# tailhook/ciruela

Measured on AMD Instinct MI355X. Metric: GiB/s block-hashed (device-resident, blocks in HBM) at 1/2/4/8 MI355X, higher is better.
Workload: dtype u64; 1 GPU; config2: 1048576 x 32768 B blocks per GPU (32 GiB), splitmix64, device-resident; blocks_per_gpu=1048576, block_size=32768, entry_point=cir_hash_chunks_dev, loader=lds-dma, parallelism=range-split x1, no collective

## Files before the change

ciruela_amd/csrc/blake2b_dev.hpp:

```cpp
#pragma once
#include <hip/hip_runtime.h>
#include <stdint.h>

#include <type_traits>

namespace cir {
namespace dev {

__device__ __forceinline__ uint32_t lo32(uint64_t x) { return (uint32_t)x; }
__device__ __forceinline__ uint32_t hi32(uint64_t x) { return (uint32_t)(x >> 32); }
__device__ __forceinline__ uint64_t mk64(uint32_t lo, uint32_t hi) {
  return ((uint64_t)hi << 32) | lo;
}
typedef uint32_t u32x2_t __attribute__((ext_vector_type(2)));
__device__ __forceinline__ uint64_t mk64_pair(uint32_t lo, uint32_t hi) {
  const u32x2_t v = {lo, hi};
  return __builtin_bit_cast(uint64_t, v);
}

__device__ __forceinline__ uint64_t xor3(uint64_t a, uint64_t b, uint64_t c) {
  return mk64(__builtin_amdgcn_bitop3_b32(lo32(a), lo32(b), lo32(c), 0x96),
              __builtin_amdgcn_bitop3_b32(hi32(a), hi32(b), hi32(c), 0x96));
}

#define CIR_IV0 0x6a09e667f3bcc908ULL
#define CIR_IV1 0xbb67ae8584caa73bULL
#define CIR_IV2 0x3c6ef372fe94f82bULL
#define CIR_IV3 0xa54ff53a5f1d36f1ULL
#define CIR_IV4 0x510e527fade682d1ULL
#define CIR_IV5 0x9b05688c2b3e6c1fULL
#define CIR_IV6 0x1f83d9abfb41bd6bULL
#define CIR_IV7 0x5be0cd19137e2179ULL
#define CIR_P0_256 0x01010020ULL

__device__ __forceinline__ void sched_fence() { __builtin_amdgcn_sched_barrier(0); }

template <int N>
__device__ __forceinline__ uint64_t rotr_lh(uint32_t l, uint32_t h) {
  if constexpr (N == 32)
    return mk64(h, l);
  else if constexpr (N < 32)
    return mk64(__builtin_amdgcn_alignbit(h, l, N), __builtin_amdgcn_alignbit(l, h, N));
  else
    return mk64(__builtin_amdgcn_alignbit(l, h, N - 32), __builtin_amdgcn_alignbit(h, l, N - 32));
}

#define CIR_XOR4(P, Q)                                            \
  tl0 = lo32(P##0) ^ lo32(Q##0); th0 = hi32(P##0) ^ hi32(Q##0);  \
  tl1 = lo32(P##1) ^ lo32(Q##1); th1 = hi32(P##1) ^ hi32(Q##1);  \
  tl2 = lo32(P##2) ^ lo32(Q##2); th2 = hi32(P##2) ^ hi32(Q##2);  \
  tl3 = lo32(P##3) ^ lo32(Q##3); th3 = hi32(P##3) ^ hi32(Q##3);
#define CIR_ROT4(P, N)              \
  P##0 = rotr_lh<N>(tl0, th0);      \
  P##1 = rotr_lh<N>(tl1, th1);      \
  P##2 = rotr_lh<N>(tl2, th2);      \
  P##3 = rotr_lh<N>(tl3, th3);
#define CIR_ADD4(P, Q) P##0 = P##0 + (Q##0); P##1 = P##1 + (Q##1); P##2 = P##2 + (Q##2); P##3 = P##3 + (Q##3);

__device__ __forceinline__ void g4(uint64_t& a0, uint64_t& a1, uint64_t& a2, uint64_t& a3,
                                   uint64_t& b0, uint64_t& b1, uint64_t& b2, uint64_t& b3,
                                   uint64_t& c0, uint64_t& c1, uint64_t& c2, uint64_t& c3,
                                   uint64_t& d0, uint64_t& d1, uint64_t& d2, uint64_t& d3,
                                   uint64_t x0, uint64_t x1, uint64_t x2, uint64_t x3,
                                   uint64_t y0, uint64_t y1, uint64_t y2, uint64_t y3) {
  uint32_t tl0, tl1, tl2, tl3, th0, th1, th2, th3;
  CIR_ADD4(a, x) CIR_ADD4(a, b)
  sched_fence();
  CIR_XOR4(d, a) CIR_ROT4(d, 32)
  sched_fence();
  CIR_ADD4(c, d)
  sched_fence();
  CIR_XOR4(b, c)
  sched_fence();
  CIR_ROT4(b, 24) CIR_ADD4(a, y) CIR_ADD4(a, b)
  sched_fence();
  CIR_XOR4(d, a)
  sched_fence();
  CIR_ROT4(d, 16) CIR_ADD4(c, d)
  sched_fence();
  CIR_XOR4(b, c)
  sched_fence();
  CIR_ROT4(b, 63)
}

#define CIR_ROUND_SM(s0, s1, s2, s3, s4, s5, s6, s7, s8, s9, s10, s11, s12, s13, s14, s15)    \
  g4(v0, v1, v2, v3, v4, v5, v6, v7, v8, v9, v10, v11, v12, v13, v14, v15, m[s0], m[s2], m[s4], \
     m[s6], m[s1], m[s3], m[s5], m[s7]);                                                       \
  g4(v0, v1, v2, v3, v5, v6, v7, v4, v10, v11, v8, v9, v15, v12, v13, v14, m[s8], m[s10],       \
     m[s12], m[s14], m[s9], m[s11], m[s13], m[s15]);

struct NoHook {
  __device__ __forceinline__ void operator()() const {}
};

template <typename Hook = NoHook>
__device__ __forceinline__ void compress_sm(uint64_t h[8], const uint64_t m[16], uint64_t t,
                                            bool last, Hook after_col0 = Hook()) {
  uint64_t v0 = h[0], v1 = h[1], v2 = h[2], v3 = h[3];
  uint64_t v4 = h[4], v5 = h[5], v6 = h[6], v7 = h[7];
  uint64_t v8 = CIR_IV0, v9 = CIR_IV1, v10 = CIR_IV2, v11 = CIR_IV3;
  uint64_t v12 = CIR_IV4 ^ t, v13 = CIR_IV5;
  uint64_t v14 = last ? ~CIR_IV6 : CIR_IV6, v15 = CIR_IV7;
  g4(v0, v1, v2, v3, v4, v5, v6, v7, v8, v9, v10, v11, v12, v13, v14, v15, m[0], m[2], m[4],
     m[6], m[1], m[3], m[5], m[7]);
  if constexpr (!std::is_same_v<Hook, NoHook>) {
    asm volatile("" : "+v"(v0), "+v"(v1), "+v"(v2), "+v"(v3), "+v"(v4), "+v"(v5), "+v"(v6),
                 "+v"(v7));
    asm volatile("" : "+v"(v8), "+v"(v9), "+v"(v10), "+v"(v11), "+v"(v12), "+v"(v13),
                 "+v"(v14), "+v"(v15));
    sched_fence();
    after_col0();
    sched_fence();
  }
  g4(v0, v1, v2, v3, v5, v6, v7, v4, v10, v11, v8, v9, v15, v12, v13, v14, m[8], m[10],
     m[12], m[14], m[9], m[11], m[13], m[15]);
  CIR_ROUND_SM(14, 10, 4, 8, 9, 15, 13, 6, 1, 12, 0, 2, 11, 7, 5, 3)
  CIR_ROUND_SM(11, 8, 12, 0, 5, 2, 15, 13, 10, 14, 3, 6, 7, 1, 9, 4)
  CIR_ROUND_SM(7, 9, 3, 1, 13, 12, 11, 14, 2, 6, 5, 10, 4, 0, 15, 8)
  CIR_ROUND_SM(9, 0, 5, 7, 2, 4, 10, 15, 14, 1, 11, 12, 6, 8, 3, 13)
  CIR_ROUND_SM(2, 12, 6, 10, 0, 11, 8, 3, 4, 13, 7, 5, 15, 14, 1, 9)
  CIR_ROUND_SM(12, 5, 1, 15, 14, 13, 4, 10, 0, 7, 6, 3, 9, 2, 8, 11)
  CIR_ROUND_SM(13, 11, 7, 14, 12, 1, 3, 9, 5, 0, 15, 4, 8, 6, 2, 10)
  CIR_ROUND_SM(6, 15, 14, 9, 11, 3, 0, 8, 12, 2, 13, 7, 1, 4, 10, 5)
  CIR_ROUND_SM(10, 2, 8, 4, 7, 6, 1, 5, 15, 11, 9, 14, 3, 12, 13, 0)
  CIR_ROUND_SM(0, 1, 2, 3, 4, 5, 6, 7, 8, 9, 10, 11, 12, 13, 14, 15)
  CIR_ROUND_SM(14, 10, 4, 8, 9, 15, 13, 6, 1, 12, 0, 2, 11, 7, 5, 3)
  sched_fence();
  h[0] = xor3(h[0], v0, v8);
  h[1] = xor3(h[1], v1, v9);
  h[2] = xor3(h[2], v2, v10);
  h[3] = xor3(h[3], v3, v11);
  h[4] = xor3(h[4], v4, v12);
  h[5] = xor3(h[5], v5, v13);
  h[6] = xor3(h[6], v6, v14);
  h[7] = xor3(h[7], v7, v15);
}

__device__ __forceinline__ void compress(uint64_t h[8], const uint64_t m[16], uint64_t t,
                                         bool last) {
  compress_sm(h, m, t, last);
}

__device__ __forceinline__ void init_state(uint64_t h[8]) {
  h[0] = CIR_IV0 ^ CIR_P0_256;
  h[1] = CIR_IV1;
  h[2] = CIR_IV2;
  h[3] = CIR_IV3;
  h[4] = CIR_IV4;
  h[5] = CIR_IV5;
  h[6] = CIR_IV6;
  h[7] = CIR_IV7;
}

__device__ __forceinline__ void load_line16(uint64_t m[16], const uint8_t* p) {
  const uint4* q = reinterpret_cast<const uint4*>(p);
#pragma unroll
  for (int k = 0; k < 8; ++k) {
    const uint4 x = q[k];
    m[2 * k] = mk64(x.x, x.y);
    m[2 * k + 1] = mk64(x.z, x.w);
  }
}

__device__ __forceinline__ void load_line_safe(uint64_t m[16], const uint8_t* p, uint32_t n) {
  const bool al4 = (reinterpret_cast<uintptr_t>(p) & 3u) == 0;
#pragma unroll
  for (int w = 0; w < 32; ++w) {
    uint32_t x = 0;
    const uint32_t b0 = 4u * w;
    if (al4 && b0 + 4u <= n) {
      x = *reinterpret_cast<const uint32_t*>(p + b0);
    } else {
#pragma unroll
      for (int k = 0; k < 4; ++k)
        if (b0 + k < n) x |= (uint32_t)p[b0 + k] << (8 * k);
    }
    if (w & 1)
      m[w >> 1] |= (uint64_t)x << 32;
    else
      m[w >> 1] = x;
  }
}

__device__ __forceinline__ void load_line_any(uint64_t m[16], const uint8_t* p, uint64_t i,
                                              uint64_t nfull, uint32_t rem, bool al16) {
  const uint8_t* q = p + (i << 7);
  if (al16 && i < nfull) {
    load_line16(m, q);
  } else {
    uint32_t n = i < nfull ? 128u : rem;
    asm volatile("" : "+v"(n));
    load_line_safe(m, q, n);
  }
}

__device__ __forceinline__ void hash_chain(const uint8_t* p, uint64_t len, uint64_t h[8]) {
  init_state(h);
  const uint32_t nfull = (uint32_t)(len >> 7);
  const uint32_t rem = (uint32_t)(len & 127u);
  const uint32_t total = nfull + ((rem != 0u || len == 0) ? 1u : 0u);
  const bool al16 = (reinterpret_cast<uintptr_t>(p) & 15u) == 0;
  uint64_t m[16];
  for (uint32_t i = 0; i < total; ++i) {
    load_line_any(m, p, i, nfull, rem, al16);
    const bool last = i + 1 == total;
    compress(h, m, last ? len : (uint64_t)(i + 1) << 7, last);
  }
}

// ... 256 lines not shown
```

ciruela_amd/csrc/kernels.hip:

```cpp
#include "kernels.hpp"

#include <algorithm>
#include <atomic>
#include <cstdlib>

#include "blake2b_dev.hpp"
#include "uniform.hpp"
#include "sha512_dev.hpp"

namespace cir {
namespace dev {

static inline unsigned grid_for(uint64_t n, uint64_t per) { return (unsigned)((n + per - 1) / per); }

__global__ __launch_bounds__(kThreads, 5) void k_uniform_glds(const uint8_t* __restrict__ data,
                                                               uint64_t bs, uint32_t lines,
                                                               uint8_t* __restrict__ out) {
  __shared__ __attribute__((aligned(16))) uint8_t lds[kWaves * kWaveLds];
  const uint32_t wave = __builtin_amdgcn_readfirstlane(threadIdx.x >> 6);
  const uint64_t blk0 = ((uint64_t)blockIdx.x * kWaves + wave) * 64u;
  uniform_glds_wave(data + blk0 * bs, bs, lines, out + blk0 * 32u, lds + wave * kWaveLds);
}

__global__ __launch_bounds__(kThreads, 4) void k_chunks(const uint8_t* __restrict__ data,
                                                         uint64_t nbytes, uint64_t bs,
                                                         uint32_t lines, uint64_t nfull,
                                                         uint32_t ngen_wg,
                                                         uint8_t* __restrict__ out) {
  __shared__ __attribute__((aligned(16))) uint8_t lds[kWaves * kWaveLds];
  if (blockIdx.x < ngen_wg) {
    if (threadIdx.x != 0) return;
    uint64_t h[8];
    hash_chain_al16(data + nfull * bs, nbytes - nfull * bs, h);
    store_digest(out + nfull * 32u, h);
    return;
  }
  const uint32_t wave = __builtin_amdgcn_readfirstlane(threadIdx.x >> 6);
  const uint64_t blk0 = ((uint64_t)(blockIdx.x - ngen_wg) * kWaves + wave) * 64u;
  if (blk0 >= nfull) return;
  const uint64_t nv = nfull - blk0;
  if (nv >= 64)
    uniform_glds_wave(data + blk0 * bs, bs, lines, out + blk0 * 32u, lds + wave * kWaveLds);
  else
    uniform_glds_wave<true>(data + blk0 * bs, bs, lines, out + blk0 * 32u, lds + wave * kWaveLds,
                            (uint32_t)nv);
}

__global__ __launch_bounds__(kThreads, 4) void k_uniform_direct(const uint8_t* __restrict__ data,
                                                                 uint64_t bs, uint32_t lines,
                                                                 uint8_t* __restrict__ out) {
  const uint64_t b = (uint64_t)blockIdx.x * kThreads + threadIdx.x;
  const uint8_t* p = data + b * bs;
  uint64_t h[8];
  init_state(h);
  uint64_t ma[16], mb[16];
  load_line16(ma, p);
  for (uint32_t i = 0; i < lines; i += 2) {
    if (i + 1 < lines) load_line16(mb, p + (uint64_t)(i + 1) * 128u);
    compress(h, ma, (uint64_t)(i + 1) * 128u, i + 1 == lines);
    if (i + 1 >= lines) break;
    if (i + 2 < lines) load_line16(ma, p + (uint64_t)(i + 2) * 128u);
    compress(h, mb, (uint64_t)(i + 2) * 128u, i + 2 == lines);
  }
  store_digest(out + b * 32u, h);
}

__global__ __launch_bounds__(kThreads, 4) void k_general(const uint8_t* __restrict__ data,
                                                          uint64_t nbytes, uint64_t bs,
                                                          uint64_t first,
                                                          const uint64_t* __restrict__ off,
                                                          const uint32_t* __restrict__ len,
                                                          const uint32_t* __restrict__ perm,
                                                          uint64_t n, uint8_t* __restrict__ out) {
  const uint64_t j = (uint64_t)blockIdx.x * kThreads + threadIdx.x;
  if (j >= n) return;
  uint64_t b, o, l;
  if (off == nullptr) {
    b = first + j;
    o = b * bs;
    const uint64_t rest = nbytes - o;
    l = rest < bs ? rest : bs;
  } else {
    b = perm ? perm[j] : j;
    o = off[b];
    l = len[b];
  }
  uint64_t h[8];
  hash_chain(data + o, l, h);
  store_digest(out + b * 32u, h);
}

__constant__ uint8_t kSigma[12][16] = {
    {0, 1, 2, 3, 4, 5, 6, 7, 8, 9, 10, 11, 12, 13, 14, 15},
    {14, 10, 4, 8, 9, 15, 13, 6, 1, 12, 0, 2, 11, 7, 5, 3},
    {11, 8, 12, 0, 5, 2, 15, 13, 10, 14, 3, 6, 7, 1, 9, 4},
    {7, 9, 3, 1, 13, 12, 11, 14, 2, 6, 5, 10, 4, 0, 15, 8},
    {9, 0, 5, 7, 2, 4, 10, 15, 14, 1, 11, 12, 6, 8, 3, 13},
    {2, 12, 6, 10, 0, 11, 8, 3, 4, 13, 7, 5, 15, 14, 1, 9},
    {12, 5, 1, 15, 14, 13, 4, 10, 0, 7, 6, 3, 9, 2, 8, 11},
    {13, 11, 7, 14, 12, 1, 3, 9, 5, 0, 15, 4, 8, 6, 2, 10},
    {6, 15, 14, 9, 11, 3, 0, 8, 12, 2, 13, 7, 1, 4, 10, 5},
    {10, 2, 8, 4, 7, 6, 1, 5, 15, 11, 9, 14, 3, 12, 13, 0},
    {0, 1, 2, 3, 4, 5, 6, 7, 8, 9, 10, 11, 12, 13, 14, 15},
    {14, 10, 4, 8, 9, 15, 13, 6, 1, 12, 0, 2, 11, 7, 5, 3}};

constexpr int kQuadWaveLds = 16 * 128;

__device__ __forceinline__ void quad_addr(uint32_t (&addr)[48], uint32_t line, uint32_t i) {
#pragma unroll
  for (int r = 0; r < 12; ++r) {
    addr[4 * r + 0] = line + 8u * kSigma[r][2 * i];
    addr[4 * r + 1] = line + 8u * kSigma[r][2 * i + 1];
    addr[4 * r + 2] = line + 8u * kSigma[r][8 + 2 * i];
    addr[4 * r + 3] = line + 8u * kSigma[r][9 + 2 * i];
  }
}

__device__ __forceinline__ uint64_t iv_lo(uint32_t i) {
  return i == 0 ? CIR_IV0 : i == 1 ? CIR_IV1 : i == 2 ? CIR_IV2 : CIR_IV3;
}
__device__ __forceinline__ uint64_t iv_hi(uint32_t i) {
  return i == 0 ? CIR_IV4 : i == 1 ? CIR_IV5 : i == 2 ? CIR_IV6 : CIR_IV7;
}

__device__ __forceinline__ void quad_init(uint32_t i, uint64_t& h0, uint64_t& h1) {
  h0 = i == 0 ? iv_lo(0) ^ CIR_P0_256 : iv_lo(i);
  h1 = iv_hi(i);
}
// ... 539 lines not shown
  __shared__ __attribute__((aligned(16))) uint8_t lds[128];
  const uint32_t i = threadIdx.x;
  if (i >= 4) return;
  uint32_t addr[48];
  quad_addr(addr, 0u, i);
  const uint64_t t0 = st[8];
  uint64_t h0 = st[i], h1 = st[4 + i];
  if (t0 == 0 && st[9] == 0) quad_init(i, h0, h1);
  quad_single(h0, h1, t0, data, n, final != 0, lds, addr, i);
  st[i] = h0;
  st[4 + i] = h1;
  if (i == 0) {
    st[8] = t0 + n;
    st[9] = 1;
  }
}

hipError_t launch_chain_step(uint64_t* st, const uint8_t* data, uint32_t n, bool final,
                             hipStream_t s) {
  hipLaunchKernelGGL(k_chain_step, dim3(1), dim3(64), 0, s, st, data, n, final ? 1 : 0);
  return hipGetLastError();
}

__global__ __launch_bounds__(kThreads) __attribute__((amdgpu_waves_per_eu(1, 1))) void k_single(
    const uint8_t* __restrict__ src, uint32_t n, uint8_t* __restrict__ scratch,
    uint8_t* __restrict__ dout) {
  __shared__ __attribute__((aligned(16))) uint8_t lds[128];
  const uint32_t nv = src == scratch ? 0u : (n + 15u) >> 4;
  const uint4* s4 = reinterpret_cast<const uint4*>(src);
  uint4* d4 = reinterpret_cast<uint4*>(scratch);
  for (uint32_t v = threadIdx.x; v < nv; v += 4u * kThreads) {
    uint4 r[4];
#pragma unroll
    for (int k = 0; k < 4; ++k) {
      const uint32_t j = v + (uint32_t)k * kThreads;
      if (j < nv) r[k] = s4[j];
    }
#pragma unroll
    for (int k = 0; k < 4; ++k) {
      const uint32_t j = v + (uint32_t)k * kThreads;
      if (j < nv) d4[j] = r[k];
    }
  }
  __threadfence_block();
  __syncthreads();
  const uint32_t i = threadIdx.x;
  if (i >= 4) return;
  __builtin_amdgcn_s_setprio(3);
  uint32_t addr[48];
  quad_addr(addr, 0u, i);
  uint64_t h0, h1;
  quad_init(i, h0, h1);
  quad_single(h0, h1, 0, scratch, n, true, lds, addr, i);
  reinterpret_cast<uint64_t*>(dout)[i] = h0;
}

hipError_t launch_single(const uint8_t* h_src, uint32_t n, uint8_t* d_scratch, uint8_t* h_out,
                         hipStream_t s) {
  hipLaunchKernelGGL(k_single, dim3(1), dim3(kThreads), 0, s, h_src, n, d_scratch, h_out);
  return hipGetLastError();
}

__global__ __launch_bounds__(kThreads, 5) void k_sha_desc(const uint8_t* __restrict__ arena,
                                                           const uint64_t* __restrict__ off,
                                                           const uint32_t* __restrict__ len,
                                                           const uint32_t* __restrict__ perm,
                                                           uint64_t n, uint8_t* __restrict__ out) {
  const uint64_t j = (uint64_t)blockIdx.x * kThreads + threadIdx.x;
  if (j >= n) return;
  const uint64_t b = perm ? perm[j] : j;
  uint64_t h[8];
  sha::chain(arena + off[b], len[b], h);
  sha::store_digest_be(out + b * 32u, h);
}

hipError_t launch_sha_desc(const uint8_t* arena, const uint64_t* off, const uint32_t* len,
                           const uint32_t* perm, uint64_t n, uint8_t* out, hipStream_t s) {
  if (n == 0) return hipSuccess;
  hipLaunchKernelGGL(k_sha_desc, dim3(grid_for(n, kThreads)), dim3(kThreads), 0, s, arena, off,
                     len, perm, n, out);
  return hipGetLastError();
}

__global__ __launch_bounds__(kThreads, 4) void k_compress_only(uint8_t* __restrict__ out,
                                                              uint32_t lines) {
  const uint64_t b = (uint64_t)blockIdx.x * kThreads + threadIdx.x;
  uint64_t h[8], m[16];
  init_state(h);
#pragma unroll
  for (int k = 0; k < 16; ++k) m[k] = b * 0x9e3779b97f4a7c15ULL + k;
  for (uint32_t i = 0; i < lines; ++i) {
    m[0] ^= i;
    compress(h, m, (uint64_t)(i + 1) * 128u, i + 1 == lines);
  }
  store_digest(out + b * 32u, h);
}

hipError_t launch_compress_only(uint64_t nlanes, uint32_t lines, uint8_t* out, hipStream_t s) {
  if (nlanes == 0) return hipSuccess;
  hipLaunchKernelGGL(k_compress_only, dim3(grid_for(nlanes, kThreads)), dim3(kThreads), 0, s, out,
                     lines);
  return hipGetLastError();
}

__global__ void k_verify(const uint8_t* __restrict__ got, const uint8_t* __restrict__ want,
                         uint64_t n, uint8_t* __restrict__ ok, uint32_t* __restrict__ nbad,
                         const uint8_t* __restrict__ flag) {
  const uint64_t b = (uint64_t)blockIdx.x * blockDim.x + threadIdx.x;
  bool bad = false;
  if (b < n) {
    const uint4* g = reinterpret_cast<const uint4*>(got + 32 * b);
    const uint4* w = reinterpret_cast<const uint4*>(want + 32 * b);
    const uint4 g0 = g[0], g1 = g[1], w0 = w[0], w1 = w[1];
    const uint32_t diff = (g0.x ^ w0.x) | (g0.y ^ w0.y) | (g0.z ^ w0.z) | (g0.w ^ w0.w) |
                          (g1.x ^ w1.x) | (g1.y ^ w1.y) | (g1.z ^ w1.z) | (g1.w ^ w1.w);
    bad = diff != 0 || (flag && flag[b]);
    if (ok) ok[b] = bad ? 0 : 1;
  }
  const uint64_t mask = __ballot(bad);
  if (nbad && (threadIdx.x & 63) == 0 && mask) atomicAdd(nbad, (uint32_t)__popcll(mask));
}

hipError_t launch_verify(const uint8_t* got, const uint8_t* want, uint64_t n, uint8_t* ok,
                         uint32_t* nbad, hipStream_t s, const uint8_t* flag) {
  if (n == 0) return hipSuccess;
  hipLaunchKernelGGL(k_verify, dim3(grid_for(n, kThreads)), dim3(kThreads), 0, s, got, want, n,
                     ok, nbad, flag);
  return hipGetLastError();
}

__global__ void k_cell_init(unsigned long long* __restrict__ first, uint32_t* __restrict__ nbad) {
  if (threadIdx.x == 0) {
    *first = ~0ull;
    if (nbad) *nbad = 0;
  }
}

__global__ void k_first_bad(const uint8_t* __restrict__ got, const uint8_t* __restrict__ want,
                            uint64_t n, uint64_t base, unsigned long long* __restrict__ first,
                            uint32_t* __restrict__ nbad, const uint8_t* __restrict__ flag) {
  const uint64_t b = (uint64_t)blockIdx.x * blockDim.x + threadIdx.x;
  bool bad = false;
  if (b < n) {
    const uint4* g = reinterpret_cast<const uint4*>(got + 32 * b);
    const uint4* w = reinterpret_cast<const uint4*>(want + 32 * b);
    const uint4 g0 = g[0], g1 = g[1], w0 = w[0], w1 = w[1];
    const uint32_t diff = (g0.x ^ w0.x) | (g0.y ^ w0.y) | (g0.z ^ w0.z) | (g0.w ^ w0.w) |
                          (g1.x ^ w1.x) | (g1.y ^ w1.y) | (g1.z ^ w1.z) | (g1.w ^ w1.w);
    bad = diff != 0 || (flag && flag[b]);
  }
  const uint64_t mask = __ballot(bad);
  if (mask && (threadIdx.x & 63) == 0) {
    atomicMin(first, (unsigned long long)(base + b + (uint64_t)__builtin_ctzll(mask)));
    if (nbad) atomicAdd(nbad, (uint32_t)__popcll(mask));
  }
}

hipError_t launch_first_bad(const uint8_t* got, const uint8_t* want, uint64_t n, uint64_t base,
                            uint64_t* first, uint32_t* nbad, hipStream_t s, const uint8_t* flag) {
  static_assert(kThreads % 64 == 0, "whole waves per workgroup");
  hipLaunchKernelGGL(k_cell_init, dim3(1), dim3(64), 0, s,
                     reinterpret_cast<unsigned long long*>(first), nbad);
  hipError_t e = hipGetLastError();
  if (e != hipSuccess || n == 0) return e;
  hipLaunchKernelGGL(k_first_bad, dim3(grid_for(n, kThreads)), dim3(kThreads), 0, s, got, want, n,
                     base, reinterpret_cast<unsigned long long*>(first), nbad, flag);
  return hipGetLastError();
}

__global__ void k_seg_init(uint8_t* __restrict__ seg_bad, uint64_t nseg,
                           uint32_t* __restrict__ nbad_seg) {
  const uint64_t i = (uint64_t)blockIdx.x * blockDim.x + threadIdx.x;
  if (i < nseg) seg_bad[i] = 0;
  if (i == 0 && nbad_seg) *nbad_seg = 0;
}

__global__ void k_seg_bad(const uint8_t* __restrict__ got, const uint8_t* __restrict__ want,
                          uint64_t n, const uint32_t* __restrict__ seg_end, uint64_t nseg,
                          uint8_t* __restrict__ seg_bad, const uint8_t* __restrict__ flag) {
  const uint64_t b = (uint64_t)blockIdx.x * blockDim.x + threadIdx.x;
  bool bad = false;
  if (b < n) {
    const uint4* g = reinterpret_cast<const uint4*>(got + 32 * b);
    const uint4* w = reinterpret_cast<const uint4*>(want + 32 * b);
// ... 58 lines not shown
    ok = diff == 0 && !(flag && flag[b]);
  }
  const uint64_t mask = __ballot(ok);
  const uint64_t miss = __ballot(b < n && !ok);
  if ((threadIdx.x & 63) == 0 && b < n) {
    have[b >> 6] = mask;
    if (nbad && miss) atomicAdd(nbad, (uint32_t)__popcll(miss));
  }
}

hipError_t launch_block_bits(const uint8_t* got, const uint8_t* want, uint64_t n, uint64_t* have,
                             uint32_t* nbad, hipStream_t s, const uint8_t* flag) {
  static_assert(kThreads % 64 == 0, "whole waves per workgroup: a wave owns one aligned word");
  hipError_t e = hipSuccess;
  if (nbad) {
    hipLaunchKernelGGL(k_count_init, dim3(1), dim3(64), 0, s, nbad);
    e = hipGetLastError();
  }
  if (e != hipSuccess || n == 0) return e;
  hipLaunchKernelGGL(k_block_bits, dim3(grid_for(n, kThreads)), dim3(kThreads), 0, s, got, want, n,
                     reinterpret_cast<unsigned long long*>(have), nbad, flag);
  return hipGetLastError();
}

__device__ __forceinline__ uint64_t splitmix64_at(uint64_t seed, uint64_t k) {
  uint64_t z = seed + (k + 1) * 0x9e3779b97f4a7c15ULL;
  z = (z ^ (z >> 30)) * 0xbf58476d1ce4e5b9ULL;
  z = (z ^ (z >> 27)) * 0x94d049bb133111ebULL;
  return z ^ (z >> 31);
}

__global__ void k_fill_splitmix64(uint64_t* __restrict__ p, uint64_t nwords, uint64_t seed,
                                  uint64_t block_words, uint64_t first_block) {
  const uint64_t stride = (uint64_t)gridDim.x * blockDim.x;
  for (uint64_t k = (uint64_t)blockIdx.x * blockDim.x + threadIdx.x; k < nwords; k += stride) {
    uint64_t sd = seed, i = k;
    if (block_words) {
      sd = seed ^ (first_block + k / block_words);
      i = k % block_words;
    }
    p[k] = splitmix64_at(sd, i);
  }
}


hipError_t launch_uniform(Loader loader, const uint8_t* data, uint64_t bs, uint64_t nblk,
                          uint8_t* out, hipStream_t s) {
  if (nblk == 0) return hipSuccess;
  if (nblk % kThreads != 0 || bs % 128u != 0 || bs == 0) return hipErrorInvalidValue;
  const uint32_t lines = (uint32_t)(bs / 128u);
  if (loader == Loader::kGlds) {
    hipLaunchKernelGGL(k_uniform_glds, dim3(grid_for(nblk, kThreads)), dim3(kThreads), 0, s, data,
                       bs, lines, out);
  } else {
    hipLaunchKernelGGL(k_uniform_direct, dim3(grid_for(nblk, kThreads)), dim3(kThreads), 0, s,
                       data, bs, lines, out);
  }
  return hipGetLastError();
}

static uint64_t device_simds() {
  static std::atomic<uint64_t> cache[64];
  int dev = 0;
  if (hipGetDevice(&dev) != hipSuccess || dev < 0 || dev >= 64) return 1024;
  uint64_t v = cache[dev].load(std::memory_order_relaxed);
  if (v == 0) {
    int cus = 0;
    if (hipDeviceGetAttribute(&cus, hipDeviceAttributeMultiprocessorCount, dev) != hipSuccess ||
        cus <= 0)
      cus = 256;
    v = 4ull * (uint64_t)cus;
    cache[dev].store(v, std::memory_order_relaxed);
  }
  return v;
}

static bool chunks_in_quad(uint64_t nblk, uint64_t bs) {
  if (bs < 128ull * kQuadSmallMinLines || bs > 0xffffffffull) return false;
  if (nblk < kQuadSmallBatch) return true;
  const uint64_t wave_slots = 64ull * device_simds();
  return nblk > wave_slots && nblk * 8 <= wave_slots * 13;
}

hipError_t launch_chunks(const uint8_t* data, uint64_t nbytes, uint64_t bs, uint8_t* out,
                         hipStream_t s) {
  if (nbytes == 0) return hipSuccess;
  if (bs == 0) return hipErrorInvalidValue;
  const uint64_t nblk = (nbytes + bs - 1) / bs;
  if (chunks_in_quad(nblk, bs)) {
    hipLaunchKernelGGL(k_quad_chunks<>, dim3((unsigned)((nblk + 63) / 64)), dim3(kThreads), 0, s,
                       data, nbytes, bs, (uint64_t)0, nblk, out);
    return hipGetLastError();
  }
  const bool uni_ok = bs % 128u == 0 && (reinterpret_cast<uintptr_t>(data) & 15u) == 0 &&
                      bs / 128u <= 0xffffffffull && bs <= 0xffffffffull / 8u;
  if (!uni_ok)
    return launch_general_chunks(data, nbytes, bs, 0, nblk, out, s);
  const uint64_t nfull = nbytes / bs;
  const uint32_t ngen_wg = nfull < nblk ? 1u : 0u;
  const uint64_t grid = ngen_wg + grid_for(grid_for(nfull, 64), kWaves);
  if (grid > 0x7fffffffull) return hipErrorInvalidValue;
  hipLaunchKernelGGL(k_chunks, dim3((unsigned)grid), dim3(kThreads), 0, s, data, nbytes, bs,
                     (uint32_t)(bs / 128u), nfull, ngen_wg, out);
  return hipGetLastError();
}

constexpr uint64_t kRelayMaxK = 32;
constexpr uint32_t kRelayLanePad = 32768;
constexpr uint32_t kRelayQuadPad = 73 * 1024;
constexpr uint32_t kRelayDescLanePad = 64 * 1024;

constexpr uint64_t kRelayCap8 = 5;
constexpr uint32_t kRelayQuad1Seg = 32;

static bool quad_relay_fits(uint64_t extra, uint64_t qslots) { return extra * 2 <= qslots; }
static uint32_t quad_relay_min_lines(uint64_t k, uint64_t extra, uint64_t qslots) {
  return extra * 4 > qslots ? 128u : (k == 1 ? 64u : 32u);
}

struct RelayPlan {
  uint64_t base = 0, nrel = 0;
  bool quad = false;
  uint32_t pad = 0;
  uint32_t min_seg = kRelayMinSegLines;
  bool relay_first = false;
};

static bool relay_plan(uint64_t nfull, uint64_t bs, RelayPlan& p) {
  p = RelayPlan();
  if (bs % 128u != 0 || bs < 128u * 16u || bs >= (1ull << 31)) return false;
  const uint64_t simds = device_simds(), lines = bs / 128u;
  const uint64_t lane_slots = 64ull * simds, quad_slots = 16ull * simds;
  if (nfull >= lane_slots) {
    const uint64_t k = nfull / lane_slots, extra = nfull % lane_slots;
    const uint64_t cap =
        std::min(lane_slots * kRelayCap8 / 8, lane_slots * lines / relay_cap_div(lines));
    if (k > kRelayMaxK || extra == 0 || extra > cap) return false;
    p.base = nfull - extra;
    p.nrel = extra;
    p.pad = k > 2 ? kRelayLanePad : 0u;
  } else {
    const uint64_t k = nfull / quad_slots, extra = nfull % quad_slots;
    if (extra == 0 || k < 1 || !quad_relay_fits(extra, quad_slots) ||
        lines < quad_relay_min_lines(k, extra, quad_slots) ||
        (nfull >= kQuadSmallBatch && extra * 64 > quad_slots))
      return false;
    p.base = nfull - extra;
    p.nrel = extra;
    p.quad = true;
    p.pad = kRelayQuadPad;
    p.min_seg = k == 1 ? kRelayQuad1Seg : kRelayMinSegLines;
    p.relay_first = true;
  }
  if ((p.nrel + kRelayGroupChains - 1) / kRelayGroupChains > kRelayMaxGroups) return false;
  return true;
}

uint64_t relay_blocks(uint64_t nfull, uint64_t bs) {
  RelayPlan p;
  return relay_plan(nfull, bs, p) ? p.nrel : 0;
}

static bool desc_may_relay_slots(uint64_t n, uint64_t slots) {
  return n >= slots && n / slots <= kRelayMaxK && n % slots != 0 &&
         (n % slots + kRelayGroupChains - 1) / kRelayGroupChains <= kRelayMaxGroups;
}

static hipError_t launch_relay(const uint8_t* data, uint64_t bs, uint64_t b0, uint64_t nrel,
                               uint32_t min_seg, uint8_t* out, hipStream_t qs,
                               const RelayScratch& r) {
  const uint32_t lines = (uint32_t)(bs / 128u);
  const uint32_t groups = (uint32_t)((nrel + kRelayGroupChains - 1) / kRelayGroupChains);
  if (groups > r.groups) return hipErrorInvalidValue;
  const uint64_t target = device_simds();
  uint32_t nseg = (uint32_t)std::max<uint64_t>(1, target / groups);
  nseg = std::min(nseg, std::max(1u, lines / min_seg));
  uint32_t seg = ((lines + nseg - 1) / nseg + 1u) & ~1u;
  nseg = (lines + seg - 1) / seg;
  uint32_t max_polls = std::max<uint32_t>(32768u, lines * 64u);
  if (const char* v = getenv("CIR_RELAY_POLLS")) max_polls = (uint32_t)strtoul(v, nullptr, 10);
  hipLaunchKernelGGL(k_quad_relay, dim3(groups * nseg), dim3(64), 0, qs, data, bs, b0,
                     (uint32_t)nrel, groups, seg, r.flags, r.state, out, max_polls);
  hipError_t e = hipGetLastError();
  if (e != hipSuccess) return e;
  hipLaunchKernelGGL(k_quad_relay_finish, dim3(groups), dim3(64), 0, qs, data, bs, b0,
                     (uint32_t)nrel, seg, r.flags, r.state, out);
  return hipGetLastError();
}

hipError_t launch_chunks_split(const uint8_t* data, uint64_t nbytes, uint64_t bs, uint8_t* out,
                               hipStream_t s, hipStream_t qs, hipEvent_t fork, hipEvent_t join,
                               const RelayScratch* relay) {
  if (nbytes == 0) return hipSuccess;
  if (bs == 0) return hipErrorInvalidValue;
  const uint64_t nblk = (nbytes + bs - 1) / bs;
  const uint64_t nfull = nbytes / bs;
  const bool uni_ok = bs % 128u == 0 && (reinterpret_cast<uintptr_t>(data) & 15u) == 0 &&
                      bs / 128u <= 0xffffffffull && bs <= 0xffffffffull / 8u;
  const uint64_t grid = grid_for(grid_for(nfull, 64), kWaves);
  RelayPlan plan;
  if (relay && relay->flags && qs && qs != s && uni_ok && relay_plan(nfull, bs, plan)) {
    hipError_t e = hipEventRecord(fork, s);
    if (e == hipSuccess) e = hipStreamWaitEvent(qs, fork, 0);
    if (e != hipSuccess) return e;
    auto base = [&]() -> hipError_t {
      if (plan.quad)
        hipLaunchKernelGGL(k_quad_chunks<true>, dim3((unsigned)grid_for(plan.base, 64)),
                           dim3(kThreads), plan.pad, s, data, nbytes, bs, (uint64_t)0, plan.base,
                           out);
      else
        hipLaunchKernelGGL(k_chunks, dim3((unsigned)grid_for(grid_for(plan.base, 64), kWaves)),
                           dim3(kThreads), plan.pad, s, data, nbytes, bs, (uint32_t)(bs / 128u),
                           plan.base, 0u, out);
      return hipGetLastError();
    };
    auto rest = [&]() -> hipError_t {
      if (nfull < nblk) {
        hipLaunchKernelGGL(k_quad_chunks<>, dim3(1), dim3(kThreads), 0, qs, data, nbytes, bs,
                           nfull, nblk, out);
        const hipError_t e2 = hipGetLastError();
        if (e2 != hipSuccess) return e2;
      }
      return launch_relay(data, bs, plan.base, plan.nrel, plan.min_seg, out, qs, *relay);
    };
    e = plan.relay_first ? rest() : base();
    if (e == hipSuccess) e = plan.relay_first ? base() : rest();
    if (e == hipSuccess) e = hipEventRecord(join, qs);
    if (e == hipSuccess) e = hipStreamWaitEvent(s, join, 0);
    return e;
  }
  if (!qs || qs == s || chunks_in_quad(nblk, bs) || !uni_ok || nfull == nblk ||
      bs < 128ull * kQuadSmallMinLines || grid > 0x7fffffffull)
    return launch_chunks(data, nbytes, bs, out, s);
  hipError_t e = hipEventRecord(fork, s);
  if (e == hipSuccess) e = hipStreamWaitEvent(qs, fork, 0);
  if (e != hipSuccess) return e;
  hipLaunchKernelGGL(k_quad_chunks<>, dim3(1), dim3(kThreads), 0, qs, data, nbytes, bs, nfull, nblk,
                     out);
  e = hipGetLastError();
  if (e != hipSuccess) return e;
  hipLaunchKernelGGL(k_chunks, dim3((unsigned)grid), dim3(kThreads), 0, s, data, nbytes, bs,
                     (uint32_t)(bs / 128u), nfull, 0u, out);
  e = hipGetLastError();
  if (e == hipSuccess) e = hipEventRecord(join, qs);
  if (e == hipSuccess) e = hipStreamWaitEvent(s, join, 0);
  return e;
}

hipError_t launch_general_chunks(const uint8_t* data, uint64_t nbytes, uint64_t bs,
                                 uint64_t first, uint64_t n, uint8_t* out, hipStream_t s) {
  if (n == 0) return hipSuccess;
  hipLaunchKernelGGL(k_general, dim3(grid_for(n, kThreads)), dim3(kThreads), 0, s, data, nbytes,
                     bs, first, (const uint64_t*)nullptr, (const uint32_t*)nullptr,
                     (const uint32_t*)nullptr, n, out);
  return hipGetLastError();
}

hipError_t launch_general_desc(const uint8_t* arena, const uint64_t* off, const uint32_t* len,
                               const uint32_t* perm, uint64_t n, uint8_t* out, hipStream_t s) {
  if (n == 0) return hipSuccess;
  hipLaunchKernelGGL(k_general, dim3(grid_for(n, kThreads)), dim3(kThreads), 0, s, arena,
                     (uint64_t)0, (uint64_t)0, (uint64_t)0, off, len, perm, n, out);
  return hipGetLastError();
}


static hipError_t launch_desc_relay(const uint8_t* arena, const uint64_t* off,
                                    const uint32_t* len, const uint32_t* perm, uint64_t n,
                                    uint32_t* n_long, uint32_t nq, uint32_t extra,
                                    uint32_t slots, uint32_t groups, uint32_t nseg_max,
                                    uint32_t qmin, uint32_t min_seg, uint32_t cap8,
                                    uint32_t gate_target, const RelayScratch& r, uint8_t* out,
                                    hipStream_t st) {
  uint32_t polls = 0;
  if (const char* v = getenv("CIR_RELAY_POLLS"))
    polls = std::max(1u, (uint32_t)strtoul(v, nullptr, 10));
  if (gate_target) {
    hipLaunchKernelGGL(k_gate, dim3(1), dim3(64), 0, st, n_long + 3, gate_target, 600u);
    const hipError_t e = hipGetLastError();
    if (e != hipSuccess) return e;
  }
  hipLaunchKernelGGL(k_desc_relay, dim3(groups * nseg_max), dim3(64), 0, st, arena, off, len,
                     perm, n, n_long, nq, extra, slots, groups, nseg_max, polls, qmin, min_seg,
                     cap8, r.flags, r.state, out);
  hipError_t e = hipGetLastError();
  if (e != hipSuccess) return e;
  hipLaunchKernelGGL(k_desc_relay_finish, dim3(groups), dim3(64), 0, st, arena, off, len, perm, n,
                     n_long, nq, extra, slots, nseg_max, qmin, min_seg, cap8, r.flags, r.state,
                     out);
  return hipGetLastError();
}

hipError_t launch_mixed(const uint8_t* arena, const uint64_t* off, const uint32_t* len,
                        const uint32_t* perm, uint32_t* n_long, uint64_t n, uint8_t* out,
                        hipStream_t s, hipStream_t qs, hipEvent_t fork, hipEvent_t qjoin,
                        const RelayScratch* relay, const hipEvent_t* tev) {
  if (n == 0) return hipSuccess;
  auto mark = [&](int k, hipStream_t st) {
    return tev ? hipEventRecord(tev[k], st) : hipSuccess;
  };
  const uint64_t slots = 64ull * device_simds();
  const uint32_t cap8 = (uint32_t)kRelayCap8;
  uint32_t extra = 0, groups = 0, nseg_max = 1;
  if (relay && relay->flags && qs != s && desc_may_relay_slots(n, slots)) {
    extra = (uint32_t)(n % slots);
    groups = (extra + kRelayGroupChains - 1) / kRelayGroupChains;
    if (groups > relay->groups) {
      extra = 0;
    } else {
      nseg_max = (uint32_t)std::max<uint64_t>(1, device_simds() / groups);
    }
  }
  const uint64_t nq = std::min<uint64_t>((n + 63) / 64, quad_max_wg(n));
  const uint64_t lane_grid = grid_for(n, kThreads);
  if (lane_grid > 0x7fffffffull) return hipErrorInvalidValue;
  const uint32_t pace = qs != s ? kLanePace : 0u;
  const bool exclusive = n >= kQuadSmallBatch;
  const uint64_t qslots = 16ull * device_simds();
  uint32_t qextra = 0;
  if (!exclusive && relay && relay->flags && qs != s &&
      n >= qslots &&
      n % qslots != 0 && quad_relay_fits(n % qslots, qslots))
    qextra = (uint32_t)(n % qslots);
  const bool serial = !exclusive && n < kQuadSmallBatch && qextra == 0;
  const bool qs_used = qs != s && !serial;
  hipError_t e = hipEventRecord(fork, s);
// ... 106 lines not shown
```

ciruela_amd/csrc/kernels.hpp:

```cpp
#pragma once
#include <hip/hip_runtime.h>
#include <stdint.h>

namespace cir {
namespace dev {

constexpr int kThreads = 256;

enum class Loader : int { kGlds = 0, kDirect = 1 };

constexpr uint32_t kQuadMinLines = 1024;
constexpr int kQuadMaxWg = 256;

constexpr uint64_t kQuadSmallBatch = 49153;
constexpr uint32_t kQuadSmallMinLines = 8;
inline uint32_t quad_min_lines(uint64_t n) {
  return n < kQuadSmallBatch ? kQuadSmallMinLines : kQuadMinLines;
}
inline uint64_t quad_max_wg(uint64_t n) {
  return n < kQuadSmallBatch ? (n + 63) / 64 : (uint64_t)kQuadMaxWg;
}

hipError_t launch_uniform(Loader loader, const uint8_t* data, uint64_t bs, uint64_t nblk,
                          uint8_t* out, hipStream_t s);

hipError_t launch_chunks(const uint8_t* data, uint64_t nbytes, uint64_t bs, uint8_t* out,
                         hipStream_t s);

struct RelayScratch {
  uint32_t* flags = nullptr;
  uint64_t* state = nullptr;
  uint32_t groups = 0;
};
constexpr uint32_t kRelayMaxGroups = 4096;
inline size_t relay_scratch_bytes(uint32_t groups) { return (size_t)groups * (4 + 64 * 16); }

hipError_t launch_chunks_split(const uint8_t* data, uint64_t nbytes, uint64_t bs, uint8_t* out,
                               hipStream_t s, hipStream_t qs, hipEvent_t fork, hipEvent_t join,
                               const RelayScratch* relay = nullptr);
uint64_t relay_blocks(uint64_t nfull, uint64_t bs);

hipError_t launch_general_chunks(const uint8_t* data, uint64_t nbytes, uint64_t bs,
                                 uint64_t first, uint64_t n, uint8_t* out, hipStream_t s);

hipError_t launch_general_desc(const uint8_t* arena, const uint64_t* off, const uint32_t* len,
                               const uint32_t* perm, uint64_t n, uint8_t* out, hipStream_t s);

hipError_t launch_mixed(const uint8_t* arena, const uint64_t* off, const uint32_t* len,
                        const uint32_t* perm, uint32_t* n_long, uint64_t n, uint8_t* out,
                        hipStream_t s, hipStream_t qs, hipEvent_t fork, hipEvent_t qjoin,
                        const RelayScratch* relay = nullptr,
                        const hipEvent_t* tev = nullptr);

size_t order_scratch_bytes(uint64_t n);
constexpr uint32_t kLaneChainCost = 4;
hipError_t launch_order_desc(const uint32_t* len, uint64_t n, void* scratch, size_t bytes,
                             uint32_t** perm, uint32_t** n_long, hipStream_t s);

size_t bound_scratch_bytes(uint64_t n);
hipError_t launch_desc_bound(const uint64_t* off, const uint32_t* len, uint64_t n,
                             uint64_t arena_bytes, void* scratch, uint32_t* nflag,
                             uint32_t** slen, uint8_t** flag, hipStream_t s);
hipError_t launch_desc_zero(const uint8_t* flag, uint64_t n, uint8_t* out, hipStream_t s);

hipError_t launch_sha_desc(const uint8_t* arena, const uint64_t* off, const uint32_t* len,
                           const uint32_t* perm, uint64_t n, uint8_t* out, hipStream_t s);

hipError_t launch_chain_step(uint64_t* st, const uint8_t* data, uint32_t n, bool final,
                             hipStream_t s);

hipError_t launch_single(const uint8_t* h_src, uint32_t n, uint8_t* d_scratch, uint8_t* h_out,
                         hipStream_t s);

hipError_t launch_verify(const uint8_t* got, const uint8_t* want, uint64_t n, uint8_t* ok,
                         uint32_t* nbad, hipStream_t s, const uint8_t* flag = nullptr);

hipError_t launch_first_bad(const uint8_t* got, const uint8_t* want, uint64_t n, uint64_t base,
                            uint64_t* first, uint32_t* nbad, hipStream_t s,
                            const uint8_t* flag = nullptr);

hipError_t launch_seg_bad(const uint8_t* got, const uint8_t* want, uint64_t n,
                          const uint32_t* seg_end, uint64_t nseg, uint8_t* seg_bad,
                          uint32_t* nbad_seg, hipStream_t s, const uint8_t* flag = nullptr);

hipError_t launch_block_bits(const uint8_t* got, const uint8_t* want, uint64_t n, uint64_t* have,
                             uint32_t* nbad, hipStream_t s, const uint8_t* flag = nullptr);

constexpr uint32_t kJoinEmpty = 0xFFFFFFFFu;
constexpr uint64_t kJoinMaxPool = 0x7FFFFFFFull;
inline uint64_t join_table_slots(uint64_t n_pool) {
// ... 35 lines not shown
```

ciruela_amd/csrc/uniform.hpp:

```cpp
#pragma once
#include "blake2b_dev.hpp"
#include "kernels.hpp"

namespace cir {
namespace dev {

constexpr int kWaves = kThreads / 64;

constexpr int kDmaAux = 2;

constexpr int kWaveLds = 8192;

template <bool kPartial = false>
__device__ __forceinline__ void uniform_glds_wave(const uint8_t* __restrict__ wsrc, uint64_t bs,
                                                  uint32_t lines, uint8_t* __restrict__ out,
                                                  uint8_t* wl, uint32_t nv = 64) {
  const uint32_t lane = threadIdx.x & 63u;
  const uint32_t r = lane >> 3;
  uint32_t dma_lane = (uint32_t)(r * bs) + 16u * ((lane & 7u) ^ r);
  const uint32_t s = (lane ^ (lane >> 3)) & 7u;
  uint32_t rd_base = lane * 128u + 16u * s;
  const uint64_t jstride = 8u * bs;

  auto issue = [&](uint32_t i) {
    const uint8_t* line = wsrc + (uint64_t)i * 128u;
#pragma unroll
    for (int j = 0; j < 8; ++j) {
      const uint8_t* src;
      if constexpr (kPartial) {
        const uint32_t blk = min(8u * j + r, nv - 1u);
        src = line + (uint64_t)blk * bs + ((16u * ((lane & 7u) ^ r)) ^ (16u * j));
      } else {
        src = line + (uint64_t)j * jstride + (dma_lane ^ (16u * j));
      }
      __builtin_amdgcn_global_load_lds(
          (const void __attribute__((address_space(1)))*)src,
          (void __attribute__((address_space(3)))*)(wl + j * 1024), 16, 0, kDmaAux);
    }
  };

  uint64_t h[8];
  init_state(h);
  uint64_t m[16];
  issue(0);
  for (uint32_t i = 0; i < lines; ++i) {
    asm volatile("" : "+v"(rd_base), "+v"(dma_lane));
    __builtin_amdgcn_s_waitcnt(0x0070);
#pragma unroll
    for (int c = 0; c < 8; ++c) {
      const uint4 x = *reinterpret_cast<const uint4*>(wl + (rd_base ^ (16u * c)));
      m[2 * c] = mk64(x.x, x.y);
      m[2 * c + 1] = mk64(x.z, x.w);
    }
    const bool last = i + 1 == lines;
    compress_sm(h, m, (uint64_t)(i + 1) * 128u, last, [&] {
      __builtin_amdgcn_s_waitcnt(0xC07F);
      if (i + 1 < lines) issue(i + 1);
    });
  }
  if (!kPartial || lane < nv) store_digest(out + lane * 32u, h);
}

}
}
```

Baseline: 2258 GiB/s.

## Lockstep chunk-hash waves with workgroup barriers inside each BLAKE2b G step

Adds a templated 'fast' hook to the BLAKE2b G function and compression that places an s_barrier at four points inside every G4 step. A new 512-thread k_chunks variant uses this to keep all eight waves of a workgroup in phase through the compression rounds. The intent is to make the waves' ALU work and LDS-DMA issue line up predictably. A host heuristic (overridable with CIR_CHUNKS_PHASE) picks it when the block count divides evenly across SIMDs; otherwise the old 256-thread kernel runs as k_chunks_free. The cost is dozens of barriers per 128-byte line, and the stricter lockstep can stall waves and hurt latency hiding.

```diff
diff --git a/ciruela_amd/csrc/blake2b_dev.hpp b/ciruela_amd/csrc/blake2b_dev.hpp
--- a/ciruela_amd/csrc/blake2b_dev.hpp
+++ b/ciruela_amd/csrc/blake2b_dev.hpp
@@ -57,27 +57,37 @@
   P##3 = rotr_lh<N>(tl3, th3);
 #define CIR_ADD4(P, Q) P##0 = P##0 + (Q##0); P##1 = P##1 + (Q##1); P##2 = P##2 + (Q##2); P##3 = P##3 + (Q##3);
 
+struct NoHook {
+  __device__ __forceinline__ void operator()() const {}
+};
+
+template <typename Fast = NoHook>
 __device__ __forceinline__ void g4(uint64_t& a0, uint64_t& a1, uint64_t& a2, uint64_t& a3,
                                    uint64_t& b0, uint64_t& b1, uint64_t& b2, uint64_t& b3,
                                    uint64_t& c0, uint64_t& c1, uint64_t& c2, uint64_t& c3,
                                    uint64_t& d0, uint64_t& d1, uint64_t& d2, uint64_t& d3,
                                    uint64_t x0, uint64_t x1, uint64_t x2, uint64_t x3,
-                                   uint64_t y0, uint64_t y1, uint64_t y2, uint64_t y3) {
+                                   uint64_t y0, uint64_t y1, uint64_t y2, uint64_t y3,
+                                   Fast fast = Fast()) {
   uint32_t tl0, tl1, tl2, tl3, th0, th1, th2, th3;
   CIR_ADD4(a, x) CIR_ADD4(a, b)
   sched_fence();
+  fast();
   CIR_XOR4(d, a) CIR_ROT4(d, 32)
   sched_fence();
   CIR_ADD4(c, d)
   sched_fence();
+  fast();
   CIR_XOR4(b, c)
   sched_fence();
   CIR_ROT4(b, 24) CIR_ADD4(a, y) CIR_ADD4(a, b)
   sched_fence();
+  fast();
   CIR_XOR4(d, a)
   sched_fence();
   CIR_ROT4(d, 16) CIR_ADD4(c, d)
   sched_fence();
+  fast();
   CIR_XOR4(b, c)
   sched_fence();
   CIR_ROT4(b, 63)
@@ -88,21 +98,23 @@
      m[s6], m[s1], m[s3], m[s5], m[s7]);                                                       \
   g4(v0, v1, v2, v3, v5, v6, v7, v4, v10, v11, v8, v9, v15, v12, v13, v14, m[s8], m[s10],       \
      m[s12], m[s14], m[s9], m[s11], m[s13], m[s15]);
-
-struct NoHook {
-  __device__ __forceinline__ void operator()() const {}
-};
-
-template <typename Hook = NoHook>
+#define CIR_ROUND_SM_F(F, s0, s1, s2, s3, s4, s5, s6, s7, s8, s9, s10, s11, s12, s13, s14, s15) \
+  g4(v0, v1, v2, v3, v4, v5, v6, v7, v8, v9, v10, v11, v12, v13, v14, v15, m[s0], m[s2], m[s4], \
+     m[s6], m[s1], m[s3], m[s5], m[s7], F);                                                    \
+  g4(v0, v1, v2, v3, v5, v6, v7, v4, v10, v11, v8, v9, v15, v12, v13, v14, m[s8], m[s10],       \
+     m[s12], m[s14], m[s9], m[s11], m[s13], m[s15], F);
+
+template <typename Hook = NoHook, typename Fast = NoHook>
 __device__ __forceinline__ void compress_sm(uint64_t h[8], const uint64_t m[16], uint64_t t,
-                                            bool last, Hook after_col0 = Hook()) {
+                                            bool last, Hook after_col0 = Hook(),
+                                            Fast fast = Fast()) {
   uint64_t v0 = h[0], v1 = h[1], v2 = h[2], v3 = h[3];
   uint64_t v4 = h[4], v5 = h[5], v6 = h[6], v7 = h[7];
   uint64_t v8 = CIR_IV0, v9 = CIR_IV1, v10 = CIR_IV2, v11 = CIR_IV3;
   uint64_t v12 = CIR_IV4 ^ t, v13 = CIR_IV5;
   uint64_t v14 = last ? ~CIR_IV6 : CIR_IV6, v15 = CIR_IV7;
   g4(v0, v1, v2, v3, v4, v5, v6, v7, v8, v9, v10, v11, v12, v13, v14, v15, m[0], m[2], m[4],
-     m[6], m[1], m[3], m[5], m[7]);
+     m[6], m[1], m[3], m[5], m[7], fast);
   if constexpr (!std::is_same_v<Hook, NoHook>) {
     asm volatile("" : "+v"(v0), "+v"(v1), "+v"(v2), "+v"(v3), "+v"(v4), "+v"(v5), "+v"(v6),
                  "+v"(v7));
@@ -113,18 +125,18 @@
     sched_fence();
   }
   g4(v0, v1, v2, v3, v5, v6, v7, v4, v10, v11, v8, v9, v15, v12, v13, v14, m[8], m[10],
-     m[12], m[14], m[9], m[11], m[13], m[15]);
-  CIR_ROUND_SM(14, 10, 4, 8, 9, 15, 13, 6, 1, 12, 0, 2, 11, 7, 5, 3)
-  CIR_ROUND_SM(11, 8, 12, 0, 5, 2, 15, 13, 10, 14, 3, 6, 7, 1, 9, 4)
-  CIR_ROUND_SM(7, 9, 3, 1, 13, 12, 11, 14, 2, 6, 5, 10, 4, 0, 15, 8)
-  CIR_ROUND_SM(9, 0, 5, 7, 2, 4, 10, 15, 14, 1, 11, 12, 6, 8, 3, 13)
-  CIR_ROUND_SM(2, 12, 6, 10, 0, 11, 8, 3, 4, 13, 7, 5, 15, 14, 1, 9)
-  CIR_ROUND_SM(12, 5, 1, 15, 14, 13, 4, 10, 0, 7, 6, 3, 9, 2, 8, 11)
-  CIR_ROUND_SM(13, 11, 7, 14, 12, 1, 3, 9, 5, 0, 15, 4, 8, 6, 2, 10)
-  CIR_ROUND_SM(6, 15, 14, 9, 11, 3, 0, 8, 12, 2, 13, 7, 1, 4, 10, 5)
-  CIR_ROUND_SM(10, 2, 8, 4, 7, 6, 1, 5, 15, 11, 9, 14, 3, 12, 13, 0)
-  CIR_ROUND_SM(0, 1, 2, 3, 4, 5, 6, 7, 8, 9, 10, 11, 12, 13, 14, 15)
-  CIR_ROUND_SM(14, 10, 4, 8, 9, 15, 13, 6, 1, 12, 0, 2, 11, 7, 5, 3)
+     m[12], m[14], m[9], m[11], m[13], m[15], fast);
+  CIR_ROUND_SM_F(fast, 14, 10, 4, 8, 9, 15, 13, 6, 1, 12, 0, 2, 11, 7, 5, 3)
+  CIR_ROUND_SM_F(fast, 11, 8, 12, 0, 5, 2, 15, 13, 10, 14, 3, 6, 7, 1, 9, 4)
+  CIR_ROUND_SM_F(fast, 7, 9, 3, 1, 13, 12, 11, 14, 2, 6, 5, 10, 4, 0, 15, 8)
+  CIR_ROUND_SM_F(fast, 9, 0, 5, 7, 2, 4, 10, 15, 14, 1, 11, 12, 6, 8, 3, 13)
+  CIR_ROUND_SM_F(fast, 2, 12, 6, 10, 0, 11, 8, 3, 4, 13, 7, 5, 15, 14, 1, 9)
+  CIR_ROUND_SM_F(fast, 12, 5, 1, 15, 14, 13, 4, 10, 0, 7, 6, 3, 9, 2, 8, 11)
+  CIR_ROUND_SM_F(fast, 13, 11, 7, 14, 12, 1, 3, 9, 5, 0, 15, 4, 8, 6, 2, 10)
+  CIR_ROUND_SM_F(fast, 6, 15, 14, 9, 11, 3, 0, 8, 12, 2, 13, 7, 1, 4, 10, 5)
+  CIR_ROUND_SM_F(fast, 10, 2, 8, 4, 7, 6, 1, 5, 15, 11, 9, 14, 3, 12, 13, 0)
+  CIR_ROUND_SM_F(fast, 0, 1, 2, 3, 4, 5, 6, 7, 8, 9, 10, 11, 12, 13, 14, 15)
+  CIR_ROUND_SM_F(fast, 14, 10, 4, 8, 9, 15, 13, 6, 1, 12, 0, 2, 11, 7, 5, 3)
   sched_fence();
   h[0] = xor3(h[0], v0, v8);
   h[1] = xor3(h[1], v1, v9);
diff --git a/ciruela_amd/csrc/kernels.hip b/ciruela_amd/csrc/kernels.hip
--- a/ciruela_amd/csrc/kernels.hip
+++ b/ciruela_amd/csrc/kernels.hip
@@ -22,11 +22,41 @@
   uniform_glds_wave(data + blk0 * bs, bs, lines, out + blk0 * 32u, lds + wave * kWaveLds);
 }
 
-__global__ __launch_bounds__(kThreads, 4) void k_chunks(const uint8_t* __restrict__ data,
-                                                         uint64_t nbytes, uint64_t bs,
-                                                         uint32_t lines, uint64_t nfull,
-                                                         uint32_t ngen_wg,
-                                                         uint8_t* __restrict__ out) {
+__global__ __launch_bounds__(kChunkThreads, 4) void k_chunks(const uint8_t* __restrict__ data,
+                                                              uint64_t nbytes, uint64_t bs,
+                                                              uint32_t lines, uint64_t nfull,
+                                                              uint32_t ngen_wg,
+                                                              uint8_t* __restrict__ out) {
+  __shared__ __attribute__((aligned(16))) uint8_t lds[kChunkWaves * kWaveLds];
+  if (blockIdx.x < ngen_wg) {
+    if (threadIdx.x != 0) return;
+    uint64_t h[8];
+    hash_chain_al16(data + nfull * bs, nbytes - nfull * bs, h);
+    store_digest(out + nfull * 32u, h);
+    return;
+  }
+  if (nfull == 0) return;
+  const uint32_t wave = __builtin_amdgcn_readfirstlane(threadIdx.x >> 6);
+  uint64_t blk0 = ((uint64_t)(blockIdx.x - ngen_wg) * kChunkWaves + wave) * 64u;
+  uint32_t nv = 1, nstore = 0;
+  if (blk0 < nfull) {
+    nv = nstore = (uint32_t)min((uint64_t)64, nfull - blk0);
+  } else {
+    blk0 = nfull - 1;
+  }
+  if (nv >= 64)
+    uniform_glds_wave<false, PhaseBarrier>(data + blk0 * bs, bs, lines, out + blk0 * 32u,
+                                           lds + wave * kWaveLds);
+  else
+    uniform_glds_wave<true, PhaseBarrier>(data + blk0 * bs, bs, lines, out + blk0 * 32u,
+                                          lds + wave * kWaveLds, nv, nstore);
+}
+
+__global__ __launch_bounds__(kThreads, 4) void k_chunks_free(const uint8_t* __restrict__ data,
+                                                              uint64_t nbytes, uint64_t bs,
+                                                              uint32_t lines, uint64_t nfull,
+                                                              uint32_t ngen_wg,
+                                                              uint8_t* __restrict__ out) {
   __shared__ __attribute__((aligned(16))) uint8_t lds[kWaves * kWaveLds];
   if (blockIdx.x < ngen_wg) {
     if (threadIdx.x != 0) return;
@@ -43,7 +73,7 @@
     uniform_glds_wave(data + blk0 * bs, bs, lines, out + blk0 * 32u, lds + wave * kWaveLds);
   else
     uniform_glds_wave<true>(data + blk0 * bs, bs, lines, out + blk0 * 32u, lds + wave * kWaveLds,
-                            (uint32_t)nv);
+                            (uint32_t)nv, (uint32_t)nv);
 }
 
 __global__ __launch_bounds__(kThreads, 4) void k_uniform_direct(const uint8_t* __restrict__ data,
@@ -749,24 +779,25 @@
   return hipGetLastError();
 }
 
-__global__ __launch_bounds__(kThreads, 4) void k_compress_only(uint8_t* __restrict__ out,
-                                                              uint32_t lines) {
-  const uint64_t b = (uint64_t)blockIdx.x * kThreads + threadIdx.x;
+__global__ __launch_bounds__(kChunkThreads, 4) void k_compress_only(uint8_t* __restrict__ out,
+                                                                   uint64_t nlanes,
+                                                                   uint32_t lines) {
+  const uint64_t b = (uint64_t)blockIdx.x * kChunkThreads + threadIdx.x;
   uint64_t h[8], m[16];
   init_state(h);
 #pragma unroll
   for (int k = 0; k < 16; ++k) m[k] = b * 0x9e3779b97f4a7c15ULL + k;
   for (uint32_t i = 0; i < lines; ++i) {
     m[0] ^= i;
-    compress(h, m, (uint64_t)(i + 1) * 128u, i + 1 == lines);
-  }
-  store_digest(out + b * 32u, h);
+    compress_sm(h, m, (uint64_t)(i + 1) * 128u, i + 1 == lines, NoHook(), PhaseBarrier());
+  }
+  if (b < nlanes) store_digest(out + b * 32u, h);
 }
 
 hipError_t launch_compress_only(uint64_t nlanes, uint32_t lines, uint8_t* out, hipStream_t s) {
   if (nlanes == 0) return hipSuccess;
-  hipLaunchKernelGGL(k_compress_only, dim3(grid_for(nlanes, kThreads)), dim3(kThreads), 0, s, out,
-                     lines);
+  hipLaunchKernelGGL(k_compress_only, dim3(grid_for(nlanes, kChunkThreads)), dim3(kChunkThreads),
+                     0, s, out, nlanes, lines);
   return hipGetLastError();
 }
 
@@ -991,6 +1022,33 @@
   return nblk > wave_slots && nblk * 8 <= wave_slots * 13;
 }
 
+static bool chunks_phase_aligned(uint64_t nfull, uint32_t pad) {
+  if (const char* v = getenv("CIR_CHUNKS_PHASE")) {
+    if (v[0] == '1') return true;
+    if (v[0] == '0') return false;
+  }
+  return pad == 0 && nfull != 0 && nfull % (128ull * device_simds()) == 0;
+}
+
+static uint64_t chunks_grid(uint64_t nfull, bool phase) {
+  return grid_for(grid_for(nfull, 64), phase ? kChunkWaves : kWaves);
+}
+
+static hipError_t launch_k_chunks(const uint8_t* data, uint64_t nbytes, uint64_t bs,
+                                  uint64_t nfull, uint32_t ngen_wg, uint32_t pad, uint8_t* out,
+                                  hipStream_t s) {
+  const bool phase = chunks_phase_aligned(nfull, pad);
+  const uint64_t grid = ngen_wg + chunks_grid(nfull, phase);
+  if (grid > 0x7fffffffull) return hipErrorInvalidValue;
+  if (phase)
+    hipLaunchKernelGGL(k_chunks, dim3((unsigned)grid), dim3(kChunkThreads), pad, s, data, nbytes,
+                       bs, (uint32_t)(bs / 128u), nfull, ngen_wg, out);
+  else
+    hipLaunchKernelGGL(k_chunks_free, dim3((unsigned)grid), dim3(kThreads), pad, s, data, nbytes,
+                       bs, (uint32_t)(bs / 128u), nfull, ngen_wg, out);
+  return hipGetLastError();
+}
+
 hipError_t launch_chunks(const uint8_t* data, uint64_t nbytes, uint64_t bs, uint8_t* out,
                          hipStream_t s) {
   if (nbytes == 0) return hipSuccess;
@@ -1007,11 +1065,7 @@
     return launch_general_chunks(data, nbytes, bs, 0, nblk, out, s);
   const uint64_t nfull = nbytes / bs;
   const uint32_t ngen_wg = nfull < nblk ? 1u : 0u;
-  const uint64_t grid = ngen_wg + grid_for(grid_for(nfull, 64), kWaves);
-  if (grid > 0x7fffffffull) return hipErrorInvalidValue;
-  hipLaunchKernelGGL(k_chunks, dim3((unsigned)grid), dim3(kThreads), 0, s, data, nbytes, bs,
-                     (uint32_t)(bs / 128u), nfull, ngen_wg, out);
-  return hipGetLastError();
+  return launch_k_chunks(data, nbytes, bs, nfull, ngen_wg, 0, out, s);
 }
 
 constexpr uint64_t kRelayMaxK = 32;
@@ -1106,7 +1160,7 @@
   const uint64_t nfull = nbytes / bs;
   const bool uni_ok = bs % 128u == 0 && (reinterpret_cast<uintptr_t>(data) & 15u) == 0 &&
                       bs / 128u <= 0xffffffffull && bs <= 0xffffffffull / 8u;
-  const uint64_t grid = grid_for(grid_for(nfull, 64), kWaves);
+  const uint64_t grid = chunks_grid(nfull, false);
   RelayPlan plan;
   if (relay && relay->flags && qs && qs != s && uni_ok && relay_plan(nfull, bs, plan)) {
     hipError_t e = hipEventRecord(fork, s);
@@ -1118,9 +1172,7 @@
                            dim3(kThreads), plan.pad, s, data, nbytes, bs, (uint64_t)0, plan.base,
                            out);
       else
-        hipLaunchKernelGGL(k_chunks, dim3((unsigned)grid_for(grid_for(plan.base, 64), kWaves)),
-                           dim3(kThreads), plan.pad, s, data, nbytes, bs, (uint32_t)(bs / 128u),
-                           plan.base, 0u, out);
+        return launch_k_chunks(data, nbytes, bs, plan.base, 0u, plan.pad, out, s);
       return hipGetLastError();
     };
     auto rest = [&]() -> hipError_t {
@@ -1148,9 +1200,7 @@
                      out);
   e = hipGetLastError();
   if (e != hipSuccess) return e;
-  hipLaunchKernelGGL(k_chunks, dim3((unsigned)grid), dim3(kThreads), 0, s, data, nbytes, bs,
-                     (uint32_t)(bs / 128u), nfull, 0u, out);
-  e = hipGetLastError();
+  e = launch_k_chunks(data, nbytes, bs, nfull, 0u, 0, out, s);
   if (e == hipSuccess) e = hipEventRecord(join, qs);
   if (e == hipSuccess) e = hipStreamWaitEvent(s, join, 0);
   return e;
diff --git a/ciruela_amd/csrc/kernels.hpp b/ciruela_amd/csrc/kernels.hpp
--- a/ciruela_amd/csrc/kernels.hpp
+++ b/ciruela_amd/csrc/kernels.hpp
@@ -6,6 +6,7 @@
 namespace dev {
 
 constexpr int kThreads = 256;
+constexpr int kChunkThreads = 512;
 
 enum class Loader : int { kGlds = 0, kDirect = 1 };
 
diff --git a/ciruela_amd/csrc/uniform.hpp b/ciruela_amd/csrc/uniform.hpp
--- a/ciruela_amd/csrc/uniform.hpp
+++ b/ciruela_amd/csrc/uniform.hpp
@@ -7,14 +7,21 @@
 
 constexpr int kWaves = kThreads / 64;
 
+constexpr int kChunkWaves = kChunkThreads / 64;
+
+struct PhaseBarrier {
+  __device__ __forceinline__ void operator()() const { __builtin_amdgcn_s_barrier(); }
+};
+
 constexpr int kDmaAux = 2;
 
 constexpr int kWaveLds = 8192;
 
-template <bool kPartial = false>
+template <bool kPartial = false, typename Fast = NoHook>
 __device__ __forceinline__ void uniform_glds_wave(const uint8_t* __restrict__ wsrc, uint64_t bs,
                                                   uint32_t lines, uint8_t* __restrict__ out,
-                                                  uint8_t* wl, uint32_t nv = 64) {
+                                                  uint8_t* wl, uint32_t nv = 64,
+                                                  uint32_t nstore = 64) {
   const uint32_t lane = threadIdx.x & 63u;
   const uint32_t r = lane >> 3;
   uint32_t dma_lane = (uint32_t)(r * bs) + 16u * ((lane & 7u) ^ r);
@@ -53,12 +60,15 @@
       m[2 * c + 1] = mk64(x.z, x.w);
     }
     const bool last = i + 1 == lines;
-    compress_sm(h, m, (uint64_t)(i + 1) * 128u, last, [&] {
-      __builtin_amdgcn_s_waitcnt(0xC07F);
-      if (i + 1 < lines) issue(i + 1);
-    });
+    compress_sm(
+        h, m, (uint64_t)(i + 1) * 128u, last,
+        [&] {
+          __builtin_amdgcn_s_waitcnt(0xC07F);
+          if (i + 1 < lines) issue(i + 1);
+        },
+        Fast());
   }
-  if (!kPartial || lane < nv) store_digest(out + lane * 32u, h);
+  if (!kPartial || lane < nstore) store_digest(out + lane * 32u, h);
 }
 
 }
```

Measured after the change: 2415 GiB/s (median of 6 runs). +6.9%, better.
